# jhollowed/PyTEMDiags

Hardware: AMD Instinct MI355X
Metric: grid-points/sec through full TEM pipeline (ncol*nlev*nt) (higher is better)
Workload: dtype f64; 1 GPU; ne120 (777602 cols) x 72 lev x 30 snapshots per GPU, L=50, 1-degree zonal grid (M=180), ten GM16 Table-A1 outputs; ncol=777602, nlev=72, nt=30, sweeps=latitude-class, single sweep, mirror_paired_sweeps=True

## Files before the change

### include/temx.h

```cpp
#ifndef TEMX_H
#define TEMX_H

#include <stdint.h>

#ifdef __cplusplus
extern "C" {
#endif

typedef struct temx_plan temx_plan;

enum { TEMX_F64 = 0, TEMX_F32 = 1 };

enum {
  TEMX_OK = 0,
  TEMX_EINVAL = -1,
  TEMX_EHIP = -2,
  TEMX_ENOMEM = -3,
  TEMX_ERANK = -4,
  TEMX_ESTATE = -5,
  TEMX_EUNSUPPORTED = -6,
  TEMX_EINTERNAL = -7
};

enum {
  TEMX_DEFER_FINALIZE = 1,
  TEMX_NO_SYMMETRY = 2,
  TEMX_NO_CLASSES = 4,
  TEMX_NO_QR = 8,
  TEMX_LAT_TOL_F32 = 16
};

enum {
  TEMX_OPT_FORM = 1,
  TEMX_OPT_OS_MAP = 2,
  TEMX_OPT_OP_MAP = 3,
  TEMX_OPT_OS_SUBSAMPLE = 4,
  TEMX_OPT_TRACER_ONE_PASS = 5,
  TEMX_OPT_SINGLE_SWEEP_MIN_GROUPS = 6,
  TEMX_OPT_OS_CONTRACT = 7,
  TEMX_OPT_MISSING = 8,
  TEMX_OPT_MIN_COVERAGE = 9,
  TEMX_OPT_MISSING_WEIGHT = 10,
  TEMX_OPT_LAT_BINS = 12,
  TEMX_OPT_BIN_DEGREE = 13,
  TEMX_OPT_OS_SYNC = 11
};
enum {
  TEMX_FORM_AUTO = -1,
  TEMX_FORM_TWO_PASS = 0,
  TEMX_FORM_CLASS_SUMS = 1,
  TEMX_FORM_SINGLE_SWEEP = 2,
  TEMX_FORM_NO_SINGLE_SWEEP = 3,
  TEMX_FORM_MASKED = 4,
  TEMX_FORM_BINNED = 5
};

enum {
  TEMX_MAT_Y0 = 0,
  TEMX_MAT_Y0P = 1,
  TEMX_MAT_GRAM = 2,
  TEMX_MAT_GINV = 3,
  TEMX_MAT_Y0INV = 4,
  TEMX_MAT_GRAM2 = 5,
  TEMX_MAT_GX = 6,
  TEMX_MAT_GSUB = 7,
  TEMX_MAT_COVERAGE = 8
};

enum {
  TEMX_R_VTEM = 0, TEMX_R_OMEGATEM, TEMX_R_WTEM, TEMX_R_PSITEM, TEMX_R_EPFY, TEMX_R_EPFZ,
  TEMX_R_EPDIV, TEMX_R_UTENDEPFD, TEMX_R_UTENDVTEM, TEMX_R_UTENDWTEM, TEMX_NRESULTS
};

enum {
  TEMX_Z_UB = 0, TEMX_Z_VB, TEMX_Z_THETAB, TEMX_Z_WAPB, TEMX_Z_UPVPB, TEMX_Z_UPWAPPB,
  TEMX_Z_VPTPB, TEMX_Z_DUB_DP, TEMX_Z_DTHETAB_DP, TEMX_Z_UBCOSLAT, TEMX_Z_DUBCOSLAT_DLAT,
  TEMX_Z_PSI, TEMX_Z_PSICOSLAT, TEMX_Z_DPSICOSLAT_DLAT, TEMX_Z_DPSI_DP, TEMX_Z_INT_VBDP,
// ... 127 lines not shown
```

### pytemdiags_amd/_lib.py

```python
from __future__ import annotations

import ctypes as C
import os

_HERE = os.path.dirname(os.path.abspath(__file__))
LIB_PATH = os.environ.get("TEMX_LIB") or os.path.join(_HERE, "libtemx.so")

ABI_VERSION = 402
F64, F32 = 0, 1
DEFER_FINALIZE = 1
NO_SYMMETRY = 2
NO_CLASSES = 4
NO_QR = 8
LAT_TOL_F32 = 16
MAT_Y0, MAT_Y0P, MAT_GRAM, MAT_GINV, MAT_Y0INV, MAT_GRAM2, MAT_GX, MAT_GSUB = 0, 1, 2, 3, 4, 5, 6, 7
MAT_COVERAGE = 8
OPT_FORM, OPT_OS_MAP, OPT_OP_MAP, OPT_OS_SUBSAMPLE, OPT_TRACER_ONE_PASS, OPT_SINGLE_SWEEP_MIN_GROUPS, OPT_OS_CONTRACT = 1, 2, 3, 4, 5, 6, 7
OPT_MISSING, OPT_MIN_COVERAGE, OPT_MISSING_WEIGHT = 8, 9, 10
OPT_OS_SYNC = 11
OPT_LAT_BINS, OPT_BIN_DEGREE = 12, 13
LAT_BINS_ALLOWED = (128, 256, 512, 1024, 2048)
LAT_BINS_DEFAULT = 512
MISSING_MODES = {"raise": 0, "mask": 1}
FORM_AUTO, FORM_TWO_PASS, FORM_CLASS_SUMS, FORM_SINGLE_SWEEP, FORM_NO_SINGLE_SWEEP = -1, 0, 1, 2, 3
FORM_MASKED = 4
FORM_BINNED = 5
FORM_NAMES = {FORM_TWO_PASS: "two-pass", FORM_CLASS_SUMS: "class-sums", FORM_SINGLE_SWEEP: "single-sweep",
              FORM_MASKED: "masked", FORM_BINNED: "binned"}
FORMS = {"auto": FORM_AUTO, "two-pass": FORM_TWO_PASS, "class-sums": FORM_CLASS_SUMS,
         "single-sweep": FORM_SINGLE_SWEEP, "no-single-sweep": FORM_NO_SINGLE_SWEEP}

RESULT_NAMES = ("vtem", "omegatem", "wtem", "psitem", "epfy", "epfz", "epdiv",
                "utendepfd", "utendvtem", "utendwtem")
ZONAL_NAMES = ("ub", "vb", "thetab", "wapb", "upvpb", "upwappb", "vptpb", "dub_dp", "dthetab_dp",
               "ubcoslat", "dubcoslat_dlat", "psi", "psicoslat", "dpsicoslat_dlat", "dpsi_dp",
               "int_vbdp")
EDDY_NAMES = ("up", "vp", "thetap", "wapp", "upvp", "upwapp", "vptp")
TRACER_RESULT_NAMES = ("etfy", "etfz", "etdiv", "qtendetfd", "qtendvtem", "qtendwtem")
TRACER_ZONAL_NAMES = ("qb", "qpvpb", "qpwappb", "dqb_dp", "qbcoslat", "dqbcoslat_dlat")
TRACER_EDDY_NAMES = ("qp", "qpvp", "qpwapp")

ERRORS = {0: "TEMX_OK", -1: "TEMX_EINVAL", -2: "TEMX_EHIP", -3: "TEMX_ENOMEM", -4: "TEMX_ERANK",
          -5: "TEMX_ESTATE", -6: "TEMX_EUNSUPPORTED", -7: "TEMX_EINTERNAL"}

_vp, _i, _i64, _dp, _u64 = C.c_void_p, C.c_int, C.c_int64, C.POINTER(C.c_double), C.c_uint64
SIGNATURES = [
    ("temx_version", _i, []),
    ("temx_last_error", C.c_char_p, []),
    ("temx_device_count", _i, []),
    ("temx_plan_create", _i, [C.POINTER(_vp), _i, _i64, _i, _i, _dp, _dp, _i]),
    ("temx_plan_finalize", _i, [_vp, _dp]),
    ("temx_plan_refine", _i, [_vp, _dp]),
# ... 114 lines not shown
```

### pytemdiags_amd/csrc/kernels_op2.hpp

```cpp
#pragma once
#include "kernels_op.hpp"

namespace temx {

template <int NA, int NB>
struct OpwSlot {
  double sd[2][NA][64];
  double y[NB * 16];
};

template <int TBS, int NA>
__device__ __forceinline__ void opw_round(const OpwSlot<NA, 2 * TBS>* slots, int par, int t0, int nbw,
                                          uint32_t yoff, int lane, double (&acc)[NA][(TBS + 1) / 2]) {
  asm volatile("s_waitcnt lgkmcnt(0)\n\ts_barrier" ::: "memory");
#pragma unroll
  for (int j = 0; j < 4; ++j) {
    double b[NA];
#pragma unroll
    for (int f = 0; f < NA; ++f) b[f] = slots[j].sd[par][f][lane];
#pragma unroll
    for (int tl = 0; tl < (TBS + 1) / 2; ++tl)
      if (tl < nbw) {
        const double ya = slots[j].y[(t0 + tl) * 16 + yoff];
#pragma unroll
// ... 548 lines not shown
#endif
template <typename T> struct RowLoad;
template <> struct RowLoad<double> {
  static __device__ __forceinline__ void ld(double& dst, uint32_t voff, uint64_t sbase) {
    asm volatile("global_load_dwordx2 %0, %1, %2 " TEMX_ROWLOAD_MOD : "=v"(dst) : "v"(voff), "s"(sbase) : "memory");
  }
};
template <> struct RowLoad<float> {
  static __device__ __forceinline__ void ld(float& dst, uint32_t voff, uint64_t sbase) {
    asm volatile("global_load_dword %0, %1, %2 " TEMX_ROWLOAD_MOD : "=v"(dst) : "v"(voff), "s"(sbase) : "memory");
  }
};
__device__ __forceinline__ double temx_rcp_count(double n) {
  double r = __builtin_amdgcn_rcp(n);
  return __builtin_fma(__builtin_fma(-n, r, 1.0), r, r);
}
template <int N, typename T>
__device__ __forceinline__ void row_wait(T& a, T& b, T& c, T& d) {
  asm volatile("s_waitcnt vmcnt(%4)" : "+v"(a), "+v"(b), "+v"(c), "+v"(d) : "n"(N) : "memory");
}
template <int N, typename T>
__device__ __forceinline__ void row_wait(T& a, T& b, T& c) {
  asm volatile("s_waitcnt vmcnt(%3)" : "+v"(a), "+v"(b), "+v"(c) : "n"(N) : "memory");
}
template <typename T>
__device__ __forceinline__ void row_touch(T& a) {
  asm volatile("" : "+v"(a)::"memory");
}

constexpr int HANDOFF_LOOKS = 1 << 22;
__device__ __forceinline__ uint32_t handoff_look(const uint32_t* ctr) {
  return __hip_atomic_load(ctr, __ATOMIC_RELAXED, __HIP_MEMORY_SCOPE_WORKGROUP);
}
template <typename T, int TBS, int TBX, int NBR, int PD, int KIND = 0, int SYNC = 0>
__global__ void __launch_bounds__(256, 1)
sweep_osr_kernel(FieldPtrs<4> fp, int64_t D, int K, int KX, const double* __restrict__ ycx,
                 const int4* __restrict__ crow, const int2* __restrict__ csplit,
                 const double* __restrict__ colscale, const double* __restrict__ rho, int K4,
                 double* __restrict__ px, double* __restrict__ pp, int nsplit, int ndt, int* __restrict__ hstat) {
  using KD = OsKind<KIND>;
  constexpr int NF = KD::NF, NFX = KD::NFX, NP = KD::NP;
  constexpr int NBX = 2 * TBX;
  constexpr int YE = NBX * 16;
  constexpr int YJ = (YE + 255) / 256;
  constexpr int MB = CLS_MB;
  constexpr int NCH = 4;
  constexpr int NV = 2 * (NF + NP);
  constexpr int NPR = KD::NPR, NPL = NP - NPR;
  static_assert(NBR <= TBS && TBS <= TBX, "reference degree <= L <= 2L");
  static_assert(YJ <= 2, "Y quarter per thread");
  static_assert((PD - 1) * CLS_MB * KD::NF + (CLS_MB - 1) * KD::NF + 2 <= 63, "the ring is counted in vmcnt (6 bits)");
  extern __shared__ double lds[];
  int split, dq;
  if (!wg_work((ndt + 3) / 4, nsplit, split, dq)) return;
  const int tid = threadIdx.x;
  const int wave = uniform_wave(), lane = tid & 63;
  const int c = lane & 15, g = lane >> 4;
  const int64_t colr = (int64_t)dq * 64 + lane < D ? (int64_t)dq * 64 + lane : D - 1;
  const uint32_t colb32 = (uint32_t)colr * (uint32_t)sizeof(T);
  const int dt = dq * 4 + wave;
  const int64_t d = (int64_t)dt * 16 + c;
  const bool dvalid = dt < ndt && d < D;
  const int64_t dcl = dvalid ? d : D - 1;
  const int b0 = __builtin_amdgcn_readfirstlane(csplit[split].x);
  const int b1 = __builtin_amdgcn_readfirstlane(csplit[split + 1].x);
  int grp = __builtin_amdgcn_readfirstlane(csplit[split].y);
  const uint32_t aoff_p = (uint32_t)(g * 4 + (lane & 3));
  const uint32_t aoff_r = (uint32_t)((lane & 3) * 4 + g);
  double* ybase = lds;
  double* cn = lds + 2 * YE;
  double* cb = lds + 2 * YE + 16 + wave * (NF * 2 * NBR * 64) + lane;
  double* apl = lds + 2 * YE + 16 + 4 * (NF * 2 * NBR * 64) + wave * (NPL * 2 * TBS * 64) + lane;
  double* ex = lds + 2 * YE + 16 + 4 * (NF * 2 * NBR * 64) + 4 * (NPL * 2 * TBS * 64);
  double* exw = ex + wave * 64 + lane;
  const double* exr = ex + g * 64 + wave * 16 + c;
  uint32_t* hctr = reinterpret_cast<uint32_t*>(ex + NV * 256);
  const double sth = (KD::TF >= 0 && colscale != nullptr) ? colscale[colr] : 1.0;
  if constexpr (SYNC != 0) {
    if (tid < 2) hctr[tid] = 0u;
    __syncthreads();
  }
#pragma unroll
  for (int i = 0; i < NPL * 2 * TBS; ++i) apl[i * 64] = 0.0;
  double apr[NPR > 0 ? NPR : 1][2 * TBS];
// ... 1 lines not shown
  for (int k = 0; k < (NPR > 0 ? NPR : 1); ++k)
#pragma unroll
    for (int t = 0; t < 2 * TBS; ++t) apr[k][t] = 0.0;
#pragma unroll
  for (int f = 0; f < NF; ++f)
#pragma unroll
    for (int tb = 0; tb < 2 * NBR; ++tb) {
      const int l = tb < NBR ? 2 * (4 * tb + g) : 2 * (4 * (tb - NBR) + g) + 1;
      const double v = rho[((int64_t)f * K4 + (l < K ? l : K - 1)) * D + dcl];
      cb[(f * 2 * NBR + tb) * 64] = l < K ? v : 0.0;
    }
  uint64_t fbase[NF];
#pragma unroll
  for (int f = 0; f < NF; ++f) fbase[f] = reinterpret_cast<uint64_t>(fp.p[f]);
  { double sth_ready = sth; asm volatile("" : "+v"(sth_ready)); }

  double ax[NFX][NBX];
#pragma unroll
  for (int f = 0; f < NFX; ++f)
#pragma unroll
    for (int t = 0; t < NBX; ++t) ax[f][t] = 0.0;
  double s[NF], q[NP], x0[NF], cnt = 0.0;
  double sN[NF], qN[NP], x0N[NF], cntN = 0.0;
#pragma unroll
  for (int f = 0; f < NF; ++f) s[f] = x0[f] = sN[f] = x0N[f] = 0.0;
#pragma unroll
  for (int k = 0; k < NP; ++k) q[k] = qN[k] = 0.0;
  bool north_open = false, prev_south = false;
  const uint32_t rowbytes = (uint32_t)D * (uint32_t)sizeof(T);

  T xb[PD][MB][NF];
  int er[PD][MB];
  double ys[YJ];
  const uint32_t yoff32[2] = {(uint32_t)(tid < YE ? tid : 0) * 8u, (uint32_t)(tid + 256 < YE ? tid + 256 : 0) * 8u};
  auto load_ys = [&](int gi) __attribute__((always_inline)) {
#pragma unroll
    for (int j = 0; j < YJ; ++j) RowLoad<double>::ld(ys[j], yoff32[j], reinterpret_cast<uint64_t>(ycx) + (uint64_t)gi * (YE * 8));
  };
  auto issue = [&](auto pc, const int4 rv) __attribute__((always_inline)) {
    constexpr int P = decltype(pc)::value;
    er[P][0] = rv.x; er[P][1] = rv.y; er[P][2] = rv.z; er[P][3] = rv.w;
#pragma unroll
    for (int j = 0; j < MB; ++j) {
      const uint64_t off = (uint64_t)(uint32_t)(er[P][j] & CLS_ROWMASK) * rowbytes;
#pragma unroll
      for (int f = 0; f < NF; ++f) RowLoad<T>::ld(xb[P][j][f], colb32, fbase[f] + off);
    }
  };
  double dS[NFX][2], dP[NP][2];
  const double* yprev = ybase;
  int ycur = 0;
  int left = 0;
#pragma unroll
  for (int f = 0; f < NFX; ++f) dS[f][0] = dS[f][1] = 0.0;
#pragma unroll
  for (int k = 0; k < NP; ++k) dP[k][0] = dP[k][1] = 0.0;
  auto pending_chunk = [&](auto cc) __attribute__((always_inline)) {
    constexpr int C = decltype(cc)::value;
#pragma unroll
    for (int t = C * NBX / NCH; t < (C + 1) * NBX / NCH; ++t) {
      const double ya = yprev[t * 16 + aoff_p];
#pragma unroll
      for (int f = 0; f < NFX; ++f) ax[f][t] = TEMX_MFMA4(ya, dS[f][t < TBX ? 0 : 1], ax[f][t]);
      const int tp = t < TBX ? t : t - TBX;
      if (tp < TBS) {
        const int ta = t < TBX ? tp : TBS + tp;
#pragma unroll
        for (int k = 0; k < NPR; ++k) apr[k][ta] = TEMX_MFMA4(ya, dP[k][t < TBX ? 0 : 1], apr[k][ta]);
        if constexpr (NPL > 0) {
          double v[NPL > 0 ? NPL : 1];
// ... 53 lines not shown
      m2[1][f] -= E[f] - O[f];
    }
#pragma unroll
    for (int f = 0; f < NFX; ++f) {
      const double SNf = nN * m2[0][f], SSf = nS * m2[1][f];
      dS[f][0] = SNf + SSf;
      dS[f][1] = SNf - SSf;
    }
#pragma unroll
    for (int k = 0; k < NP; ++k) {
      const double PNk = c2[0][k] + nN * m2[0][KD::pa(k)] * m2[0][KD::pb(k)];
      const double PSk = c2[1][k] + nS * m2[1][KD::pa(k)] * m2[1][KD::pb(k)];
      dP[k][0] = PNk + PSk;
      dP[k][1] = PNk - PSk;
    }
    yprev = yw;
    left = NCH;
  };
  uint32_t hgen = 0;
  bool hpend = false;
  int hfail = 0;
  const double* ypend = ybase;
  auto handoff_wait = [&](const uint32_t* ctr, uint32_t seen, uint32_t need, int code) __attribute__((always_inline)) {
    seen = (uint32_t)__builtin_amdgcn_readfirstlane((int)seen);
    if (seen >= need || hfail != 0) return;
#pragma unroll 1
    for (int n = 0; n < HANDOFF_LOOKS; ++n) {
      __builtin_amdgcn_s_sleep(1);
      seen = (uint32_t)__builtin_amdgcn_readfirstlane((int)handoff_look(ctr));
      if (seen >= need) return;
    }
    hfail = code;
  };
  int4 rn;
  auto step = [&](auto posc, int b) __attribute__((always_inline)) {
    constexpr int POS = decltype(posc)::value % NCH;
    constexpr int P = decltype(posc)::value % PD;
    uint32_t seen = 0;
    if constexpr (SYNC != 0) {
      if (hpend) seen = handoff_look(&hctr[0]);
    }
    {
      const int4 r1 = rn;
      rn = crow[(int64_t)(b + PD) * 4 + wave];
      issue(std::integral_constant<int, (P + PD - 1) % PD>{}, r1);
    }
    if constexpr (SYNC != 0) {
      if (hpend) {
        if (left > 0)
          static_for<NCH>([&](auto cc) __attribute__((always_inline)) {
            if (((decltype(cc)::value - POS) & (NCH - 1)) < left) pending_chunk(cc);
          });
        handoff_wait(&hctr[0], seen, 4u * hgen, 1);
        tile_role(ypend);
        hpend = false;
      }
    }
    if (left > 0) {
      if (!(TEMX_OS_SKIP & 1)) pending_chunk(std::integral_constant<int, POS>{});
      --left;
    }
    static_assert(NF == 4 || NF == 3, "row_wait has forms for 3 and 4 fields");
    static_for<MB>([&](auto jc) __attribute__((always_inline)) {
      constexpr int j = decltype(jc)::value;
      constexpr int NW = (PD - 1) * MB * NF + (MB - 1 - j) * NF;
      if constexpr (NF == 4) row_wait<NW>(xb[P][j][0], xb[P][j][1], xb[P][j][2], xb[P][j][3]);
      else row_wait<NW>(xb[P][j][0], xb[P][j][1], xb[P][j][2]);
    });
#pragma unroll
    for (int j = 0; j < YJ; ++j) row_touch(ys[j]);
    const int fl = er[P][0] >> 27;
    const bool south = (fl & (CLS_SOUTH << 1)) != 0;
    if ((fl & (CLS_FIRST << 1)) || (south && !prev_south)) {
      if (south && north_open) park_north();
      north_open = !south;
#pragma unroll
      for (int f = 0; f < NF; ++f) x0[f] = (double)xb[P][0][f];
    }
    prev_south = south;
#pragma unroll
    for (int j = 0; j < ((TEMX_OS_SKIP & 4) ? 0 : MB); ++j) {
      const double w = er[P][j] < 0 ? 0.0 : 1.0;
      double dx[NF];
#pragma unroll
      for (int f = 0; f < NF; ++f) dx[f] = (double)xb[P][j][f] - x0[f];
#pragma unroll
      for (int f = 0; f < NF; ++f) s[f] += w * dx[f];
#pragma unroll
      for (int k = 0; k < NP; ++k) q[k] += (w * dx[KD::pa(k)]) * dx[KD::pb(k)];
      cnt += w;
    }
    if (fl & (CLS_LAST << 1)) {
      prev_south = false;
      if (north_open) park_north();
      north_open = false;
      uint32_t seen_done = 0;
      if constexpr (SYNC == 0) {
        if (left > 0)
          static_for<NCH>([&](auto cc) __attribute__((always_inline)) {
            if (((decltype(cc)::value - POS - 1) & (NCH - 1)) < left) pending_chunk(cc);
          });
      } else {
        seen_done = handoff_look(&hctr[1]);
      }
      const double rnN = cntN > 0.0 ? temx_rcp_count(cntN) : 0.0, rnS = cnt > 0.0 ? temx_rcp_count(cnt) : 0.0;
      double val[NV];
#pragma unroll
      for (int f = 0; f < NF; ++f) {
        const double sc = f == KD::TF ? sth : 1.0;
        val[f] = (sN[f] * rnN + x0N[f]) * sc;
        val[NF + NP + f] = (s[f] * rnS + x0[f]) * sc;
      }
#pragma unroll
      for (int k = 0; k < NP; ++k) {
        const double sc = k == KD::TP ? sth : 1.0;
        val[NF + k] = (qN[k] - sN[KD::pa(k)] * sN[KD::pb(k)] * rnN) * sc;
        val[2 * NF + NP + k] = (q[k] - s[KD::pa(k)] * s[KD::pb(k)] * rnS) * sc;
      }
      if constexpr (SYNC == 0) {
        if (!(TEMX_OS_SKIP & 8)) asm volatile("s_waitcnt lgkmcnt(0)\n\ts_barrier" ::: "memory");
      } else {
        handoff_wait(&hctr[1], seen_done, 4u * hgen, 2);
      }
      ycur ^= 1;
      double* yw = ybase + ycur * YE;
#pragma unroll
      for (int v = 0; v < NV; ++v) exw[v * 256] = val[v];
      if (lane == 0) {
        cn[wave] = cntN;
        cn[4 + wave] = cnt;
      }
#pragma unroll
      for (int j = 0; j < YJ; ++j)
        if (tid + 256 * j < YE) yw[tid + 256 * j] = ys[j];
      if constexpr (SYNC == 0) {
        if (!(TEMX_OS_SKIP & 8)) asm volatile("s_waitcnt lgkmcnt(0)\n\ts_barrier" ::: "memory");
      } else {
        asm volatile("s_waitcnt lgkmcnt(0)" ::: "memory");
        if (lane == 0) __hip_atomic_fetch_add(&hctr[0], 1u, __ATOMIC_RELAXED, __HIP_MEMORY_SCOPE_WORKGROUP);
        ++hgen;
        hpend = true;
        ypend = yw;
      }
      ++grp;
      load_ys(grp);
      if constexpr (SYNC == 0) tile_role(yw);
#pragma unroll
      for (int f = 0; f < NF; ++f) s[f] = sN[f] = 0.0;
#pragma unroll
      for (int k = 0; k < NP; ++k) q[k] = qN[k] = 0.0;
      cnt = cntN = 0.0;
    }
  };

  if (b0 < b1) {
    load_ys(grp);
    rn = crow[(int64_t)b0 * 4 + wave];
    static_for<PD - 1>([&](auto kc) __attribute__((always_inline)) {
      constexpr int k = decltype(kc)::value;
      const int4 r0 = rn;
      rn = crow[(int64_t)(b0 + k + 1) * 4 + wave];
      issue(kc, r0);
    });
    constexpr int UNR = PD % 4 == 0 ? PD : PD % 2 == 0 ? 2 * PD : 4 * PD;
    for (int b = b0; b < b1; b += UNR)
      static_for<UNR>([&](auto kc) __attribute__((always_inline)) {
        constexpr int k = decltype(kc)::value;
        if (k == 0 || b + k < b1) step(kc, b + k);
      });
    asm volatile("s_waitcnt vmcnt(0)" ::: "memory");
  }
  if constexpr (SYNC != 0) {
    if (hpend) {
      if (left > 0) {
        const int first = (b1 - b0) & (NCH - 1);
        static_for<NCH>([&](auto cc) __attribute__((always_inline)) {
          if (((decltype(cc)::value - first) & (NCH - 1)) < left) pending_chunk(cc);
        });
      }
      handoff_wait(&hctr[0], handoff_look(&hctr[0]), 4u * hgen, 1);
      tile_role(ypend);
    }
    if (hfail != 0 && lane == 0) atomicOr(hstat, hfail);
  }
  if (left > 0) {
    const int first = (b1 - b0) & (NCH - 1);
    static_for<NCH>([&](auto cc) __attribute__((always_inline)) {
      if (((decltype(cc)::value - first) & (NCH - 1)) < left) pending_chunk(cc);
    });
  }
  if (dvalid) {
#pragma unroll
    for (int f = 0; f < NFX; ++f)
#pragma unroll
      for (int t = 0; t < NBX; ++t) {
        const int l = symx_harm<TBX>(t, g);
        if (l < (pp != nullptr ? KX : K4)) px[(((int64_t)split * NFX + f) * KX + l) * D + d] = ax[f][t];
      }
#pragma unroll
    for (int k = 0; k < NP; ++k)
#pragma unroll
      for (int t = 0; t < 2 * TBS; ++t) {
        const int l = sym_harm<TBS>(t, g);
        if (pp != nullptr && l < K) pp[(((int64_t)split * NP + k) * K + l) * D + d] = k < NPR ? apr[k < NPR ? k : 0][t] : apl[((k < NPR ? 0 : k - NPR) * 2 * TBS + t) * 64];
      }
  }
}

#ifndef TEMX_OS2_STAGGER
#define TEMX_OS2_STAGGER 0
#endif
#ifndef TEMX_OS2_ACC32
#define TEMX_OS2_ACC32 1
#endif
// ... 703 lines not shown
```

### pytemdiags_amd/csrc/temx.hip

```cpp
#include "../../include/temx.h"
#include "../../include/temx_vert.h"
#include "../../include/temx_layout.h"
#include "../../include/temx_ingest.h"
#include "../../include/temx_clim.h"
#include "../../include/temx_mtracer.h"
#include "../../include/temx_nclim.h"
#include "../../include/temx_gclim.h"
#include "../include/temx_mgclim.h"
#include "../include/temx_wave.h"
#include "../include/temx_tfilt.h"

#include <hip/hip_runtime.h>

#include <algorithm>
#include <cmath>
#include <cstdarg>
#include <cstdio>
#include <cstdlib>
#include <cstring>
#include <map>
#include <mutex>
#include <new>
#include <stdexcept>
#include <string>
// ... 115 lines not shown
  Split sp_proj1;
  bool sym = false;
  int TBS = 0;
  int64_t npair = 0, npg = 0, npg_alloc = 0;
  DevBuf rows, ysym;
  Split sp_sproj4, sp_sproj1, sp_seddy;
  Split sp_proj4, sp_eddy;
  bool cls = false;
  int64_t cgroups = 0, cbatches = 0, ncls = 0;
  int64_t cls_max_side = 0;
  std::vector<int> gbatch0;
  DevBuf crow, ycls;
  std::map<int, DevBuf> csplits;
  Split sp_cproj4, sp_cproj1, sp_ceddy, sp_cflux;
  bool os_built = false, os_on = false;
  bool os_valid = false;
  DevBuf Axq, rho_t;
  int TBX = 0, KX = 0, KR = 0, NQ = 0;
  std::vector<double> h_xc, h_cnt;
  std::vector<int> h_crow;
  std::vector<int> sgbatch0;
  int64_t sgroups = 0, sbatches = 0;
  DevBuf ycx, ycx_s, crow_s, rho, rho0, gaunt , wq2, Gx, Gsinv, Ax , Axs ;
  std::vector<double> h_G_own;
  std::vector<double> h_Gx_own;
  std::vector<double> h_Gx, h_Gs;
  std::vector<double> h_T, h_Ginv, h_G, h_Yq;
  DevBuf oscblk, osAt, osAb, osAtq, osAbq, Bqp;
  OscMats osc{};
  bool osc_lds = false;
  int opt_os_contract = -1;
  bool os_barrier = false;
  int opt_os_sync = -1;
  int os_keep = 32;
  int64_t tD = 0, tnt = 0, tt0 = 0;
  int opt_form = -1, opt_os_map = -1, opt_op_map = -1, opt_tracer_one_pass = -1, opt_single_sweep_min_groups = -1;
  bool os_tile = false, op_tile = false;
  bool no_qr = false;
  DevBuf side_crow[2][2], side_gfirst[2][2];
  std::map<int, DevBuf> csplits_s;
  Split sp_os, sp_os_s;
  Split sp_copw;
  bool lcls = false, lone = false, xb_valid = false;
  DevBuf ycls_l, pbuf;
  int64_t ycls_lstride = 0;
  Split sp_lflux;
  bool onepass = false, op_valid = false;
  bool c4_valid = false;
  DevBuf csum, ccnt;
  DevBuf Pq;
  DevBuf csq, Pq2;
  bool tq_valid = false;
  DevBuf partial;
  DevBuf opB, opC;
  int opt_missing = 0, opt_min_cov = 500, opt_miss_w = 10;
  bool miss_built = false;
  bool miss_valid = false;
  int64_t miss_cov_D = -1;
  int NE = 0, NQM = 0;
  DevBuf eblk;
  DevBuf mtab;
  DevBuf mB, mC, mCcov, mcov, mZ;
  bool mt_valid = false;
  DevBuf mtB, mtB2, mtC, mtCcov, mtz;
  int opt_lat_bins = 0;
  int bin_J = 0, bin_KP = 0;
// ... 648 lines not shown
  constexpr int NBR = OS_NBR;
  constexpr int PDv = sizeof(T) == 4 ? 4 : 2;
  constexpr int DF = TEMX_OS_DEFER;
  const bool tile_map = pl->os_tile;
  double* px = partial;
  double* pp = sub ? nullptr : partial + (int64_t)sp.nsplit * KD::NFX * pl->KX * pl->D;
  int rc = TEMX_OK;
  const bool listed = dispatch_strict(OsPairs{}, pl->TBS, pl->TBX, rc, [&](auto pair) {
    constexpr int TBSv = decltype(pair)::first, TBXv = decltype(pair)::second;
    if constexpr (KIND == 3) {
      if (tile_map) return fail(TEMX_EUNSUPPORTED, "two tracers per sweep: row-map sweeps only");
    }
    if constexpr (KIND != 3) if (tile_map) {
      constexpr size_t lds = sweep_os_lds(TBSv, TBXv, KD::NF, KD::NP, KD::NPR, DF);
      return launch_lds<sweep_os_kernel<T, TBSv, TBXv, NBR, PDv, KIND, DF>>(pl->device, grid, block, lds, st, fp, pl->D,
          pl->K, pl->KX, sub ? pl->ycx_s.d() : pl->ycx.d(), static_cast<const int4*>(sub ? pl->crow_s.p : pl->crow.p), cuts,
          pl->colscale.d(), rho, pl->KR, px, pp, sp.nsplit, sp.ndt);
    }
    if (sizeof(T) == 4) {
      if (pl->cls_max_side > 8 * TEMX_F32_SIDE_CAP)
        return fail(TEMX_EUNSUPPORTED, "single sweep of fp32 fields: a latitude class of this plan has %lld members on one "
                    "side, and the sweep sums a side in fp32; create the plan with TEMX_LAT_TOL_F32",
                    (long long)pl->cls_max_side);
      constexpr size_t lds = sweep_os2_lds(TBSv, TBXv, KD::NF, KD::NP, KD::NPR, DF);
      const int si = sub ? 1 : 0;
      return launch_lds<sweep_os2_kernel<float, TBSv, TBXv, NBR, 2, KIND>>(
          pl->device, grid, dim3(512), lds, st, fp, pl->D, pl->K, pl->KX, sub ? pl->ycx_s.d() : pl->ycx.d(),
          static_cast<const int4*>(pl->side_crow[si][0].p), static_cast<const int4*>(pl->side_crow[si][1].p),
          static_cast<const int*>(pl->side_gfirst[si][0].p), static_cast<const int*>(pl->side_gfirst[si][1].p),
          cuts, pl->colscale.d(), rho, pl->KR, px, pp, sp.nsplit, sp.ndt);
    }
    constexpr size_t lds = sweep_osr_lds(TBSv, TBXv, KD::NF, KD::NP, KD::NPR, DF);
    static_assert(lds <= 163840, "the single sweep's workgroup fits the LDS of a compute unit");
    auto go = [&](auto handoff) {
      return launch_lds<sweep_osr_kernel<double, TBSv, TBXv, NBR, 2, KIND, decltype(handoff)::value>>(pl->device, grid,
          block, lds, st, fp, pl->D, pl->K, pl->KX, sub ? pl->ycx_s.d() : pl->ycx.d(),
          static_cast<const int4*>(sub ? pl->crow_s.p : pl->crow.p), cuts, pl->colscale.d(), rho, pl->KR, px, pp, sp.nsplit,
          sp.ndt, static_cast<int*>(pl->flag.p) + 1);
    };
    return pl->os_barrier ? go(Int<0>{}) : go(Int<1>{});
  });
  return listed ? rc : fail(TEMX_EUNSUPPORTED, "single-sweep form: no instantiation for L = %d", pl->L);
}

template <int KIND>
static int launch_sweep_os(temx_plan* pl, const FieldPtrs<4>& fp, int dtype, bool sub, const double* rho, double* partial,
                           const Split& sp, hipStream_t st) {
  return dtype == TEMX_F64 ? launch_sweep_os_t<double, KIND>(pl, fp, sub, rho, partial, sp, st)
                           : launch_sweep_os_t<float, KIND>(pl, fp, sub, rho, partial, sp, st);
}

static bool os_supported(const temx_plan* pl) {
  return os_supported(pl->cls, pl->large, pl->weighted, pl->qbasis, !pl->h_crow.empty(), pl->TBS, pl->L);
}

static bool os_active(const temx_plan* pl, int dtype) {
  (void)dtype;
  return pl->os_on;
}

static void set_tail(temx_plan* pl, int64_t t0, int64_t nts) {
  if (pl->tt0 != t0 || pl->tnt != nts) pl->c4_valid = pl->os_valid = pl->op_valid = pl->tq_valid = pl->xb_valid = false;
  pl->tt0 = t0;
  pl->tnt = nts;
  pl->tD = (int64_t)pl->nlev * nts;
}
static inline bool tail_is_whole(const temx_plan* pl) { return pl->tt0 == 0 && pl->tnt == pl->nt; }

static int tem_stage3_impl(temx_plan* pl, const double* B3, double* results, double* zonal, hipStream_t st);
static int tem_epilogue(temx_plan* pl, double* results, double* zonal, hipStream_t st);
static int bin_project_op(temx_plan* pl, const void* A, int dtype, int64_t D, double* B, hipStream_t st);
static int bin_zonal_mean(temx_plan* pl, const void* A, int dtype, int64_t D, double* out, int native, hipStream_t st);
static int miss_check(const temx_plan* pl);
// ... 1291 lines not shown
  if (!pl || !B || !out) return fail(TEMX_EINVAL, "null argument");
  if (!pl->finalized) return fail(TEMX_ESTATE, "plan not finalised");
  HIPCHK(hipSetDevice(pl->device));
  int rc;
  if (!native) return launch_solve(pl, B, 1, D, nullptr, out, S_(stream));
  if ((rc = pl->opC.ensure((size_t)pl->K4 * D * 8))) return rc;
  if ((rc = launch_solve(pl, B, 1, D, pl->opC.d(), nullptr, S_(stream)))) return rc;
  return launch_recon(pl, D, pl->opC.d(), out, S_(stream));
} TEMX_CATCH

int temx_zonal_mean(temx_plan* pl, const void* A, int dtype, int64_t D, double* out, int native,
                    void* stream) try {
  if (!pl || !A || !out) return fail(TEMX_EINVAL, "null argument");
  if (!pl->finalized) return fail(TEMX_ESTATE, "plan not finalised");
  if (miss_mode(pl)) return miss_zonal_mean(pl, A, dtype, D, out, native, S_(stream));
  if (bin_mode(pl)) return bin_zonal_mean(pl, A, dtype, D, out, native, S_(stream));
  int rc = pl->opB.ensure((size_t)pl->K * std::max<int64_t>(D, 1) * 8);
  if (rc) return rc;
  if ((rc = temx_project(pl, A, dtype, D, pl->opB.d(), stream))) return rc;
  return temx_zonal_mean_from_sums(pl, pl->opB.d(), D, out, native, stream);
} TEMX_CATCH

static FormChoice form_choice(const temx_plan* pl) {
  return form_choice(pl->opt_form, bin_mode(pl), getenv("TEMX_TWO_PASS"), getenv("TEMX_ONE_PASS"), getenv("TEMX_SINGLE_SWEEP"));
}
static bool tile_map(int opt, const char* env) {
  if (const char* e = getenv(env)) return !strcmp(e, "tile");
  return opt == 1;
}
static bool os_barrier_wanted(const temx_plan* pl) {
  if (const char* e = getenv("TEMX_OS_SYNC")) return !strcmp(e, "barrier");
  return pl->opt_os_sync == 1;
}
static bool tracer_one_pass_wanted(const temx_plan* pl) {
  if (const char* e = getenv("TEMX_TRACER_ONE_PASS")) return e[0] == '1';
  return pl->opt_tracer_one_pass == 1;
}

static int bin_check(const temx_plan* pl);
static int bin_set_tem(temx_plan* pl);

int temx_plan_configure(temx_plan* pl, int option, int value) try {
  if (!pl) return fail(TEMX_EINVAL, "null plan");
  switch (option) {
    case TEMX_OPT_FORM:
      if (value < -1 || value > TEMX_FORM_NO_SINGLE_SWEEP) return fail(TEMX_EINVAL, "TEMX_OPT_FORM: unknown form %d", value);
      pl->opt_form = value;
      break;
    case TEMX_OPT_OS_MAP: pl->opt_os_map = value; break;
    case TEMX_OPT_OP_MAP: pl->opt_op_map = value; break;
    case TEMX_OPT_TRACER_ONE_PASS: pl->opt_tracer_one_pass = value; break;
    case TEMX_OPT_OS_SUBSAMPLE:
      if (value < 4) return fail(TEMX_EINVAL, "TEMX_OPT_OS_SUBSAMPLE: at least 4 class-groups");
      if (pl->os_built && value != pl->os_keep) return fail(TEMX_ESTATE, "the single-sweep tables of this plan are built: set the subsample before temx_plan_set_tem");
      pl->os_keep = value;
      break;
    case TEMX_OPT_SINGLE_SWEEP_MIN_GROUPS: pl->opt_single_sweep_min_groups = value; break;
    case TEMX_OPT_OS_CONTRACT: pl->opt_os_contract = value; break;
    case TEMX_OPT_MISSING:
      if (value != 0 && value != 1) return fail(TEMX_EINVAL, "TEMX_OPT_MISSING: 0 (raise) or 1 (mask), got %d", value);
      if (value == 1) {
        if (bin_mode(pl)) return fail(TEMX_EUNSUPPORTED, "missing-value mode is not available while latitude bins are in effect (TEMX_OPT_LAT_BINS)");
        if (int rc = miss_check(pl)) return rc;
      }
      pl->opt_missing = value;
      pl->miss_valid = false;
      break;
    case TEMX_OPT_MIN_COVERAGE:
      if (value < 0 || value > 1000) return fail(TEMX_EINVAL, "TEMX_OPT_MIN_COVERAGE: per mille in 0..1000, got %d", value);
      pl->opt_min_cov = value;
      break;
    case TEMX_OPT_MISSING_WEIGHT:
      if (value < 4 || value > 14) return fail(TEMX_EINVAL, "TEMX_OPT_MISSING_WEIGHT: tau = 10^-value, value in 4..14, got %d", value);
      pl->opt_miss_w = value;
      break;
    case TEMX_OPT_OS_SYNC:
      if (value != 0 && value != 1) return fail(TEMX_EINVAL, "TEMX_OPT_OS_SYNC: 0 (flags) or 1 (barriers), got %d", value);
      pl->opt_os_sync = value;
      break;
    case TEMX_OPT_LAT_BINS: {
      const int B = value == -1 ? BIN_DEFAULT : value;
      if (B != 0) {
        if (!bin_count_ok(B)) return fail(TEMX_EINVAL, "TEMX_OPT_LAT_BINS: 0 (off), -1 (default, %d) or one of 128, 256, 512, 1024, 2048, got %d", BIN_DEFAULT, value);
        if (int rc = bin_check(pl)) return rc;
        if (bin_degree(pl->L, B) == 0)
          return fail(TEMX_EINVAL, "TEMX_OPT_LAT_BINS: (L, B) = (%d, %d): no Chebyshev degree up to %d keeps the basis rows to %.0e; use more bins",
                      pl->L, B, BIN_MAX_DEGREE, BIN_BOUND);
      }
      pl->opt_lat_bins = B;
      pl->bin_J = B ? bin_degree(pl->L, B) : 0;
      break;
    }
    case TEMX_OPT_BIN_DEGREE: return fail(TEMX_EINVAL, "TEMX_OPT_BIN_DEGREE is chosen by the library (read it with temx_plan_option)");
    default: return fail(TEMX_EINVAL, "unknown option %d", option);
  }
  pl->tem = false;
  return TEMX_OK;
} TEMX_CATCH

int temx_plan_option(const temx_plan* pl, int option) try {
  if (!pl) return -1;
  switch (option) {
    case TEMX_OPT_FORM:
      if (miss_mode(pl)) return TEMX_FORM_MASKED;
      if (bin_mode(pl)) return TEMX_FORM_BINNED;
      return pl->os_on ? TEMX_FORM_SINGLE_SWEEP : ((pl->cls && pl->onepass) || (pl->lcls && pl->lone) ? TEMX_FORM_CLASS_SUMS : TEMX_FORM_TWO_PASS);
    case TEMX_OPT_OS_MAP: return tile_map(pl->opt_os_map, "TEMX_OS_MAP") ? 1 : 0;
    case TEMX_OPT_OP_MAP: return tile_map(pl->opt_op_map, "TEMX_OP_MAP") ? 1 : 0;
    case TEMX_OPT_TRACER_ONE_PASS: return tracer_one_pass_wanted(pl) ? 1 : 0;
    case TEMX_OPT_OS_SUBSAMPLE: return pl->os_keep;
    case TEMX_OPT_SINGLE_SWEEP_MIN_GROUPS: return pl->opt_single_sweep_min_groups;
    case TEMX_OPT_OS_CONTRACT: return pl->osc_lds ? 1 : 0;
    case TEMX_OPT_MISSING: return pl->opt_missing;
    case TEMX_OPT_MIN_COVERAGE: return pl->opt_min_cov;
    case TEMX_OPT_MISSING_WEIGHT: return pl->opt_miss_w;
    case TEMX_OPT_OS_SYNC: return os_barrier_wanted(pl) ? 1 : 0;
    case TEMX_OPT_LAT_BINS: return pl->opt_lat_bins;
    case TEMX_OPT_BIN_DEGREE: return pl->bin_J;
    default: return -1;
  }
} TEMX_CATCH

static bool mem_free(size_t* fr) {
  size_t tot = 0;
  return hipMemGetInfo(fr, &tot) == hipSuccess;
}

static int set_tem_large_cls(temx_plan* pl, const TemDims& d, const FormChoice& fc) {
  const LargeClsLayout l = tem_large_cls_layout(d, fc);
  size_t fr = 0;
  if (!(l.eligible && mem_free(&fr) && fits(l.csum, pl->csum.bytes, fr, l.pbuf) &&
        alloc_write_stream(pl->csum, l.csum) == TEMX_OK && pl->pbuf.ensure(l.pbuf) == TEMX_OK))
    return TEMX_OK;
  int rc;
  HIPCHK(hipMemset(pl->csum.p, 0, pl->csum.bytes));
  HIPCHK(hipMemset(pl->pbuf.p, 0, pl->pbuf.bytes));
  pl->sp_cproj4 = l.sp_cproj4;
  pl->sp_cflux = l.sp_cflux;
  pl->sp_lflux = l.sp_lflux;
  if ((rc = pl->partial.ensure(l.partial))) return rc;
  if ((rc = pl->Bs.ensure(l.Bs))) return rc;
  const int2* cuts_unused = nullptr;
  if ((rc = class_cuts_dev(pl, pl->sp_cproj4.nsplit, &cuts_unused, true))) return rc;
  pl->lone = true;
  return TEMX_OK;
}

static int set_tem_single_sweep(temx_plan* pl, const TemDims& d) {
  int rc = build_os_tables(pl);
// ... 47 lines not shown
  for (int nsub : {pl->sp_cproj4.nsplit, pl->sp_cproj1.nsplit, pl->sp_ceddy.nsplit * (8 / d.edpw())})
    if ((rc = class_cuts_dev(pl, nsub, &cuts_unused))) return rc;
  return TEMX_OK;
}

static int set_tem_sym(temx_plan* pl, const TemDims& d) {
  const SymLayout s = tem_sym_layout(d);
  pl->sp_sproj4 = s.sp_sproj4;
  pl->sp_sproj1 = s.sp_sproj1;
  pl->sp_seddy = s.sp_seddy;
  return pl->partial.ensure(s.partial);
}

int temx_plan_set_tem(temx_plan* pl, int nlev, int64_t nt, const double* p_pa_host, double p0) try {
  if (!pl || !p_pa_host) return fail(TEMX_EINVAL, "null argument");
  if (nlev < 2 || nt < 1) return fail(TEMX_EINVAL, "need nlev >= 2 and nt >= 1");
  if ((int64_t)nlev * nt >= ((int64_t)1 << 28)) return fail(TEMX_EINVAL, "nlev*nt must be < 2^28");
  if (pl->M < 2) return fail(TEMX_EINVAL, "need at least 2 zonal-mean latitudes");
  HIPCHK(hipSetDevice(pl->device));
  std::vector<double> p(p_pa_host, p_pa_host + nlev);
  for (int j = 1; j < nlev; ++j)
    if (!(p[j] > p[j - 1])) return fail(TEMX_EINVAL, "pressure must be strictly ascending (front end flips)");
  pl->tem = false;
  pl->onepass = pl->lone = pl->op_valid = pl->xb_valid = pl->tq_valid = false;
  pl->os_on = pl->os_valid = false;
  pl->miss_valid = pl->mt_valid = false;
  pl->os_tile = tile_map(pl->opt_os_map, "TEMX_OS_MAP");
  {
    const char* e = getenv("TEMX_OS_CONTRACT");
    pl->osc_lds = e ? !strcmp(e, "lds") : pl->opt_os_contract == 1;
  }
  pl->op_tile = tile_map(pl->opt_op_map, "TEMX_OP_MAP");
  pl->os_barrier = os_barrier_wanted(pl);
  pl->nlev = nlev;
  pl->nt = nt;
  pl->D = (int64_t)nlev * nt;
  pl->tD = pl->D;
  pl->tnt = nt;
  pl->tt0 = 0;
  pl->p0 = p0;
  int rc;
  const TemTables tt = tem_tables(p, nt, p0, pl->lat_out_deg);
  if ((rc = upload(pl->p, p))) return rc;
  if ((rc = upload(pl->pg, tt.pg))) return rc;
  if ((rc = upload(pl->lg, tt.lg))) return rc;
  if ((rc = upload(pl->coslat, tt.coslat))) return rc;
  if ((rc = upload(pl->fcor, tt.fcor))) return rc;
  if ((rc = upload(pl->colscale, tt.colscale))) return rc;

  const TemDims d = tem_dims(pl);
  const FormChoice fc = form_choice(pl);
  const BaseLayout b = tem_base_layout(d);
  pl->sp_proj4 = b.sp_proj4;
  pl->sp_eddy = b.sp_eddy;
  pl->sp_proj1 = b.sp_proj1;
  if ((rc = pl->partial.ensure(b.partial))) return rc;
  if ((rc = pl->B4.ensure(b.B4))) return rc;
  if ((rc = pl->B3.ensure(b.B3))) return rc;
  if ((rc = pl->C4.ensure(b.C4))) return rc;
  if ((rc = pl->zb.ensure(b.zb))) return rc;
  if ((rc = pl->partial.ensure(b.partial_unfused))) return rc;
  if (pl->lcls && (rc = set_tem_large_cls(pl, d, fc))) return rc;
  if (pl->cls && (rc = set_tem_cls(pl, d, fc))) return rc;
  if (pl->sym && (rc = set_tem_sym(pl, d))) return rc;
  if (bin_mode(pl) && (rc = bin_set_tem(pl))) return rc;
  pl->tem = true;
// ... 1600 lines not shown
```

### pytemdiags_amd/engine.py

```python
from __future__ import annotations

import ctypes as C

import numpy as np
import torch

from . import _lib
from ._lib import check

_DT = {torch.float64: _lib.F64, torch.float32: _lib.F32}


def _ptr(t):
    return C.c_void_p(t.data_ptr())


def _dbl(a):
    a = np.ascontiguousarray(a, dtype=np.float64)
    return a, a.ctypes.data_as(C.POINTER(C.c_double))


def lat_bins_value(lat_bins):
    if lat_bins is None or lat_bins is False:
        return 0
# ... 23 lines not shown
        check(self.lib.temx_plan_create(C.byref(self._h), self.device_index, self.N, self.L, self.M,
                                        plat, plat_out, (_lib.DEFER_FINALIZE if defer_finalize else 0)
                                        | (0 if symmetry else _lib.NO_SYMMETRY)
                                        | (0 if classes else _lib.NO_CLASSES)
                                        | (0 if qr else _lib.NO_QR)
                                        | (_lib.LAT_TOL_F32 if fp32_fields else 0)))
        if form is not None:
            self.configure(form=form)
        if lat_bins is not None:
            self.configure(lat_bins=lat_bins)

    @property
    def paired(self):
        return bool(self.lib.temx_plan_is_paired(self._h))

    @property
    def sweep_mode(self):
        return int(self.lib.temx_plan_sweep_mode(self._h))

    @property
    def one_pass(self):
        return bool(self.lib.temx_plan_one_pass(self._h))

    @property
    def single_sweep(self):
        return bool(self.lib.temx_plan_single_sweep(self._h))

    @property
    def tracer_one_pass(self):
        return self.one_pass and self.option(_lib.OPT_TRACER_ONE_PASS) == 1

    def configure(self, form=None, os_map=None, op_map=None, os_subsample=None, tracer_one_pass=None,
                  single_sweep_min_groups=None, os_contract=None, missing=None, min_coverage=None,
                  missing_weight=None, os_sync=None, lat_bins=None):
        def put(opt, val):
            check(self.lib.temx_plan_configure(self._h, opt, int(val)))
        if missing is not None:
            if missing not in _lib.MISSING_MODES:
                raise ValueError("missing must be 'raise' or 'mask', got %r" % (missing,))
            put(_lib.OPT_MISSING, _lib.MISSING_MODES[missing])
        if min_coverage is not None:
            mc = float(min_coverage)
            if not 0.0 <= mc <= 1.0:
                raise ValueError("min_coverage must lie in [0, 1], got %r" % (min_coverage,))
            put(_lib.OPT_MIN_COVERAGE, int(round(mc * 1000)))
        if missing_weight is not None:
            e = -np.log10(float(missing_weight))
            if not (float(missing_weight) > 0 and abs(e - round(e)) < 1e-9 and 4 <= round(e) <= 14):
                raise ValueError("missing_weight must be 10^-n with n in 4..14, got %r" % (missing_weight,))
            put(_lib.OPT_MISSING_WEIGHT, int(round(e)))
        if form is not None:
            put(_lib.OPT_FORM, _lib.FORMS[form] if isinstance(form, str) else form)
            self.form_requested = form
        for opt, val in ((_lib.OPT_OS_MAP, os_map), (_lib.OPT_OP_MAP, op_map)):
            if val is not None:
                put(opt, {"row": 0, "tile": 1}[val] if isinstance(val, str) else val)
        if os_subsample is not None:
            put(_lib.OPT_OS_SUBSAMPLE, os_subsample)
        if tracer_one_pass is not None:
            put(_lib.OPT_TRACER_ONE_PASS, 1 if tracer_one_pass else 0)
        if single_sweep_min_groups is not None:
            put(_lib.OPT_SINGLE_SWEEP_MIN_GROUPS, single_sweep_min_groups)
        if os_contract is not None:
            put(_lib.OPT_OS_CONTRACT, {"mfma": 0, "lds": 1}[os_contract] if isinstance(os_contract, str) else os_contract)
        if lat_bins is not None:
            put(_lib.OPT_LAT_BINS, lat_bins_value(lat_bins))
        if os_sync is not None:
            put(_lib.OPT_OS_SYNC, {"flags": 0, "barrier": 1}[os_sync] if isinstance(os_sync, str) else os_sync)
        self.nlev = self.nt = self.D = None

    def option(self, opt):
        return int(self.lib.temx_plan_option(self._h, int(opt)))

    @property
    def lat_bins(self):
        return self.option(_lib.OPT_LAT_BINS)

    @property
    def bin_degree(self):
        return self.option(_lib.OPT_BIN_DEGREE)

    @property
    def sweep_form(self):
        return _lib.FORM_NAMES.get(self.option(_lib.OPT_FORM), "two-pass")

    @property
    def missing(self):
        return "mask" if self.option(_lib.OPT_MISSING) == 1 else "raise"

    def coverage(self):
        D = getattr(self, "_cov_D", None) or self.D or 1
        out = torch.empty((self.M, D), dtype=torch.float64, device=self.device)
        check(self.lib.temx_get_matrix(self._h, _lib.MAT_COVERAGE, _ptr(out), self._stream()))
        return out

    def close(self):
        if getattr(self, "_h", None) is not None and self._h.value:
            self.lib.temx_plan_destroy(self._h)
            self._h = C.c_void_p()

    def __del__(self):
# ... 639 lines not shown
```

Before: 189.3 billion grid-points/s.

## Defer single-sweep group hand-over production until after next chunk issue

Adds a 'late' hand-over variant to the flag-synchronised single-sweep kernel, now the default. When a latitude group closes, the kernel no longer computes and publishes its zonal statistics and Y rows on the spot. It records a pending production, prefetches the next group's Y into a separate register set, and performs the production at the next step, after the following row loads are issued. The goal is to hide the hand-over wait and LDS writes behind in-flight memory traffic. In exchange it uses extra registers, adds scalar state, and needs more careful ordering at the kernel tail.

Result: no change. 191.7 billion grid-points/s, median of 6 (+1.3%).

```diff
diff --git a/include/temx.h b/include/temx.h
--- a/include/temx.h
+++ b/include/temx.h
@@ -43,6 +43,7 @@
   TEMX_OPT_MISSING_WEIGHT = 10,
   TEMX_OPT_LAT_BINS = 12,
   TEMX_OPT_BIN_DEGREE = 13,
+  TEMX_OPT_OS_HANDOVER = 14,
   TEMX_OPT_OS_SYNC = 11
 };
 enum {
diff --git a/pytemdiags_amd/_lib.py b/pytemdiags_amd/_lib.py
--- a/pytemdiags_amd/_lib.py
+++ b/pytemdiags_amd/_lib.py
@@ -18,6 +18,7 @@
 OPT_FORM, OPT_OS_MAP, OPT_OP_MAP, OPT_OS_SUBSAMPLE, OPT_TRACER_ONE_PASS, OPT_SINGLE_SWEEP_MIN_GROUPS, OPT_OS_CONTRACT = 1, 2, 3, 4, 5, 6, 7
 OPT_MISSING, OPT_MIN_COVERAGE, OPT_MISSING_WEIGHT = 8, 9, 10
 OPT_OS_SYNC = 11
+OPT_OS_HANDOVER = 14
 OPT_LAT_BINS, OPT_BIN_DEGREE = 12, 13
 LAT_BINS_ALLOWED = (128, 256, 512, 1024, 2048)
 LAT_BINS_DEFAULT = 512
diff --git a/pytemdiags_amd/csrc/kernels_op2.hpp b/pytemdiags_amd/csrc/kernels_op2.hpp
--- a/pytemdiags_amd/csrc/kernels_op2.hpp
+++ b/pytemdiags_amd/csrc/kernels_op2.hpp
@@ -604,7 +604,7 @@
 __device__ __forceinline__ uint32_t handoff_look(const uint32_t* ctr) {
   return __hip_atomic_load(ctr, __ATOMIC_RELAXED, __HIP_MEMORY_SCOPE_WORKGROUP);
 }
-template <typename T, int TBS, int TBX, int NBR, int PD, int KIND = 0, int SYNC = 0>
+template <typename T, int TBS, int TBX, int NBR, int PD, int KIND = 0, int SYNC = 0, int LATE = 0>
 __global__ void __launch_bounds__(256, 1)
 sweep_osr_kernel(FieldPtrs<4> fp, int64_t D, int K, int KX, const double* __restrict__ ycx,
                  const int4* __restrict__ crow, const int2* __restrict__ csplit,
@@ -622,6 +622,7 @@
   static_assert(NBR <= TBS && TBS <= TBX, "reference degree <= L <= 2L");
   static_assert(YJ <= 2, "Y quarter per thread");
   static_assert((PD - 1) * CLS_MB * KD::NF + (CLS_MB - 1) * KD::NF + 2 <= 63, "the ring is counted in vmcnt (6 bits)");
+  static_assert(LATE == 0 || SYNC != 0, "the late hand-over is a form of the flag hand-over");
   extern __shared__ double lds[];
   int split, dq;
   if (!wg_work((ndt + 3) / 4, nsplit, split, dq)) return;
@@ -689,10 +690,11 @@
   T xb[PD][MB][NF];
   int er[PD][MB];
   double ys[YJ];
+  double ysn[LATE ? YJ : 1];
   const uint32_t yoff32[2] = {(uint32_t)(tid < YE ? tid : 0) * 8u, (uint32_t)(tid + 256 < YE ? tid + 256 : 0) * 8u};
   auto load_ys = [&](int gi) __attribute__((always_inline)) {
 #pragma unroll
-    for (int j = 0; j < YJ; ++j) RowLoad<double>::ld(ys[j], yoff32[j], reinterpret_cast<uint64_t>(ycx) + (uint64_t)gi * (YE * 8));
+    for (int j = 0; j < YJ; ++j) RowLoad<double>::ld(LATE ? ysn[LATE ? j : 0] : ys[j], yoff32[j], reinterpret_cast<uint64_t>(ycx) + (uint64_t)gi * (YE * 8));
   };
   auto issue = [&](auto pc, const int4 rv) __attribute__((always_inline)) {
     constexpr int P = decltype(pc)::value;
@@ -812,13 +814,67 @@
     }
     hfail = code;
   };
+  auto produce = [&](uint32_t seen_done) __attribute__((always_inline)) {
+    const double rnN = cntN > 0.0 ? temx_rcp_count(cntN) : 0.0, rnS = cnt > 0.0 ? temx_rcp_count(cnt) : 0.0;
+    double val[NV];
+#pragma unroll
+    for (int f = 0; f < NF; ++f) {
+      const double sc = f == KD::TF ? sth : 1.0;
+      val[f] = (sN[f] * rnN + x0N[f]) * sc;
+      val[NF + NP + f] = (s[f] * rnS + x0[f]) * sc;
+    }
+#pragma unroll
+    for (int k = 0; k < NP; ++k) {
+      const double sc = k == KD::TP ? sth : 1.0;
+      val[NF + k] = (qN[k] - sN[KD::pa(k)] * sN[KD::pb(k)] * rnN) * sc;
+      val[2 * NF + NP + k] = (q[k] - s[KD::pa(k)] * s[KD::pb(k)] * rnS) * sc;
+    }
+    if constexpr (SYNC == 0) {
+      if (!(TEMX_OS_SKIP & 8)) asm volatile("s_waitcnt lgkmcnt(0)\n\ts_barrier" ::: "memory");
+    } else {
+      handoff_wait(&hctr[1], seen_done, 4u * hgen, 2);
+    }
+    ycur ^= 1;
+    double* yw = ybase + ycur * YE;
+#pragma unroll
+    for (int v = 0; v < NV; ++v) exw[v * 256] = val[v];
+    if (lane == 0) {
+      cn[wave] = cntN;
+      cn[4 + wave] = cnt;
+    }
+#pragma unroll
+    for (int j = 0; j < YJ; ++j)
+      if (tid + 256 * j < YE) yw[tid + 256 * j] = ys[j];
+    if constexpr (SYNC == 0) {
+      if (!(TEMX_OS_SKIP & 8)) asm volatile("s_waitcnt lgkmcnt(0)\n\ts_barrier" ::: "memory");
+    } else {
+      asm volatile("s_waitcnt lgkmcnt(0)" ::: "memory");
+      if (lane == 0) __hip_atomic_fetch_add(&hctr[0], 1u, __ATOMIC_RELAXED, __HIP_MEMORY_SCOPE_WORKGROUP);
+      ++hgen;
+      hpend = true;
+      ypend = yw;
+    }
+    return yw;
+  };
+  auto zero_sums = [&]() __attribute__((always_inline)) {
+#pragma unroll
+    for (int f = 0; f < NF; ++f) s[f] = sN[f] = 0.0;
+#pragma unroll
+    for (int k = 0; k < NP; ++k) q[k] = qN[k] = 0.0;
+    cnt = cntN = 0.0;
+  };
+  int hprod = 0;
   int4 rn;
   auto step = [&](auto posc, int b) __attribute__((always_inline)) {
     constexpr int POS = decltype(posc)::value % NCH;
     constexpr int P = decltype(posc)::value % PD;
-    uint32_t seen = 0;
+    uint32_t seen = 0, seen_late = 0;
     if constexpr (SYNC != 0) {
       if (hpend) seen = handoff_look(&hctr[0]);
+      if constexpr (LATE != 0) {
+        asm volatile("" : "+s"(hprod));
+        if (hprod) seen_late = handoff_look(&hctr[1]);
+      }
     }
     {
       const int4 r1 = rn;
@@ -834,6 +890,16 @@
         handoff_wait(&hctr[0], seen, 4u * hgen, 1);
         tile_role(ypend);
         hpend = false;
+        if constexpr (LATE != 0) {
+          if (hprod) seen_late = handoff_look(&hctr[1]);
+        }
+      }
+      if constexpr (LATE != 0) {
+        if (hprod) {
+          produce(seen_late);
+          zero_sums();
+          hprod = 0;
+        }
       }
     }
     if (left > 0) {
@@ -847,8 +913,16 @@
       if constexpr (NF == 4) row_wait<NW>(xb[P][j][0], xb[P][j][1], xb[P][j][2], xb[P][j][3]);
       else row_wait<NW>(xb[P][j][0], xb[P][j][1], xb[P][j][2]);
     });
-#pragma unroll
-    for (int j = 0; j < YJ; ++j) row_touch(ys[j]);
+    if constexpr (LATE != 0) {
+#pragma unroll
+      for (int j = 0; j < YJ; ++j) {
+        row_touch(ysn[j]);
+        asm volatile("v_mov_b64 %0, %1" : "=v"(ys[j]) : "v"(ysn[j]));
+      }
+    } else {
+#pragma unroll
+      for (int j = 0; j < YJ; ++j) row_touch(ys[j]);
+    }
     const int fl = er[P][0] >> 27;
     const bool south = (fl & (CLS_SOUTH << 1)) != 0;
     if ((fl & (CLS_FIRST << 1)) || (south && !prev_south)) {
@@ -874,62 +948,30 @@
       prev_south = false;
       if (north_open) park_north();
       north_open = false;
-      uint32_t seen_done = 0;
-      if constexpr (SYNC == 0) {
-        if (left > 0)
-          static_for<NCH>([&](auto cc) __attribute__((always_inline)) {
-            if (((decltype(cc)::value - POS - 1) & (NCH - 1)) < left) pending_chunk(cc);
-          });
+      if constexpr (LATE != 0) {
+        hprod = 1;
+        ++grp;
+        load_ys(grp);
+        int no = north_open, ps = prev_south;
+        asm volatile("" : "+s"(no), "+s"(ps));
+        north_open = no != 0;
+        prev_south = ps != 0;
       } else {
-        seen_done = handoff_look(&hctr[1]);
-      }
-      const double rnN = cntN > 0.0 ? temx_rcp_count(cntN) : 0.0, rnS = cnt > 0.0 ? temx_rcp_count(cnt) : 0.0;
-      double val[NV];
-#pragma unroll
-      for (int f = 0; f < NF; ++f) {
-        const double sc = f == KD::TF ? sth : 1.0;
-        val[f] = (sN[f] * rnN + x0N[f]) * sc;
-        val[NF + NP + f] = (s[f] * rnS + x0[f]) * sc;
-      }
-#pragma unroll
-      for (int k = 0; k < NP; ++k) {
-        const double sc = k == KD::TP ? sth : 1.0;
-        val[NF + k] = (qN[k] - sN[KD::pa(k)] * sN[KD::pb(k)] * rnN) * sc;
-        val[2 * NF + NP + k] = (q[k] - s[KD::pa(k)] * s[KD::pb(k)] * rnS) * sc;
-      }
-      if constexpr (SYNC == 0) {
-        if (!(TEMX_OS_SKIP & 8)) asm volatile("s_waitcnt lgkmcnt(0)\n\ts_barrier" ::: "memory");
-      } else {
-        handoff_wait(&hctr[1], seen_done, 4u * hgen, 2);
-      }
-      ycur ^= 1;
-      double* yw = ybase + ycur * YE;
-#pragma unroll
-      for (int v = 0; v < NV; ++v) exw[v * 256] = val[v];
-      if (lane == 0) {
-        cn[wave] = cntN;
-        cn[4 + wave] = cnt;
-      }
-#pragma unroll
-      for (int j = 0; j < YJ; ++j)
-        if (tid + 256 * j < YE) yw[tid + 256 * j] = ys[j];
-      if constexpr (SYNC == 0) {
-        if (!(TEMX_OS_SKIP & 8)) asm volatile("s_waitcnt lgkmcnt(0)\n\ts_barrier" ::: "memory");
-      } else {
-        asm volatile("s_waitcnt lgkmcnt(0)" ::: "memory");
-        if (lane == 0) __hip_atomic_fetch_add(&hctr[0], 1u, __ATOMIC_RELAXED, __HIP_MEMORY_SCOPE_WORKGROUP);
-        ++hgen;
-        hpend = true;
-        ypend = yw;
-      }
-      ++grp;
-      load_ys(grp);
-      if constexpr (SYNC == 0) tile_role(yw);
-#pragma unroll
-      for (int f = 0; f < NF; ++f) s[f] = sN[f] = 0.0;
-#pragma unroll
-      for (int k = 0; k < NP; ++k) q[k] = qN[k] = 0.0;
-      cnt = cntN = 0.0;
+        uint32_t seen_done = 0;
+        if constexpr (SYNC == 0) {
+          if (left > 0)
+            static_for<NCH>([&](auto cc) __attribute__((always_inline)) {
+              if (((decltype(cc)::value - POS - 1) & (NCH - 1)) < left) pending_chunk(cc);
+            });
+        } else {
+          seen_done = handoff_look(&hctr[1]);
+        }
+        double* yw = produce(seen_done);
+        ++grp;
+        load_ys(grp);
+        if constexpr (SYNC == 0) tile_role(yw);
+        zero_sums();
+      }
     }
   };
 
@@ -951,7 +993,7 @@
     asm volatile("s_waitcnt vmcnt(0)" ::: "memory");
   }
   if constexpr (SYNC != 0) {
-    if (hpend) {
+    auto take_last = [&]() __attribute__((always_inline)) {
       if (left > 0) {
         const int first = (b1 - b0) & (NCH - 1);
         static_for<NCH>([&](auto cc) __attribute__((always_inline)) {
@@ -960,6 +1002,14 @@
       }
       handoff_wait(&hctr[0], handoff_look(&hctr[0]), 4u * hgen, 1);
       tile_role(ypend);
+      hpend = false;
+    };
+    if (hpend) take_last();
+    if constexpr (LATE != 0) {
+      if (hprod) {
+        produce(handoff_look(&hctr[1]));
+        take_last();
+      }
     }
     if (hfail != 0 && lane == 0) atomicOr(hstat, hfail);
   }
diff --git a/pytemdiags_amd/csrc/temx.hip b/pytemdiags_amd/csrc/temx.hip
--- a/pytemdiags_amd/csrc/temx.hip
+++ b/pytemdiags_amd/csrc/temx.hip
@@ -171,6 +171,8 @@
   int opt_os_contract = -1;
   bool os_barrier = false;
   int opt_os_sync = -1;
+  bool os_late = false;
+  int opt_os_handover = -1;
   int os_keep = 32;
   int64_t tD = 0, tnt = 0, tt0 = 0;
   int opt_form = -1, opt_os_map = -1, opt_op_map = -1, opt_tracer_one_pass = -1, opt_single_sweep_min_groups = -1;
@@ -885,13 +887,13 @@
     }
     constexpr size_t lds = sweep_osr_lds(TBSv, TBXv, KD::NF, KD::NP, KD::NPR, DF);
     static_assert(lds <= 163840, "the single sweep's workgroup fits the LDS of a compute unit");
-    auto go = [&](auto handoff) {
-      return launch_lds<sweep_osr_kernel<double, TBSv, TBXv, NBR, 2, KIND, decltype(handoff)::value>>(pl->device, grid,
+    auto go = [&](auto handoff, auto late) {
+      return launch_lds<sweep_osr_kernel<double, TBSv, TBXv, NBR, 2, KIND, decltype(handoff)::value, decltype(late)::value>>(pl->device, grid,
           block, lds, st, fp, pl->D, pl->K, pl->KX, sub ? pl->ycx_s.d() : pl->ycx.d(),
           static_cast<const int4*>(sub ? pl->crow_s.p : pl->crow.p), cuts, pl->colscale.d(), rho, pl->KR, px, pp, sp.nsplit,
           sp.ndt, static_cast<int*>(pl->flag.p) + 1);
     };
-    return pl->os_barrier ? go(Int<0>{}) : go(Int<1>{});
+    return pl->os_barrier ? go(Int<0>{}, Int<0>{}) : pl->os_late ? go(Int<1>{}, Int<1>{}) : go(Int<1>{}, Int<0>{});
   });
   return listed ? rc : fail(TEMX_EUNSUPPORTED, "single-sweep form: no instantiation for L = %d", pl->L);
 }
@@ -2249,6 +2251,14 @@
   if (const char* e = getenv("TEMX_OS_SYNC")) return !strcmp(e, "barrier");
   return pl->opt_os_sync == 1;
 }
+constexpr int OS_HANDOVER_DEFAULT = 1;
+static bool os_late_wanted(const temx_plan* pl) {
+  if (const char* e = getenv("TEMX_OS_HANDOVER")) {
+    if (!strcmp(e, "late")) return true;
+    if (!strcmp(e, "early")) return false;
+  }
+  return (pl->opt_os_handover < 0 ? OS_HANDOVER_DEFAULT : pl->opt_os_handover) == 1;
+}
 static bool tracer_one_pass_wanted(const temx_plan* pl) {
   if (const char* e = getenv("TEMX_TRACER_ONE_PASS")) return e[0] == '1';
   return pl->opt_tracer_one_pass == 1;
@@ -2295,6 +2305,10 @@
       if (value != 0 && value != 1) return fail(TEMX_EINVAL, "TEMX_OPT_OS_SYNC: 0 (flags) or 1 (barriers), got %d", value);
       pl->opt_os_sync = value;
       break;
+    case TEMX_OPT_OS_HANDOVER:
+      if (value != 0 && value != 1) return fail(TEMX_EINVAL, "TEMX_OPT_OS_HANDOVER: 0 (early) or 1 (late), got %d", value);
+      pl->opt_os_handover = value;
+      break;
     case TEMX_OPT_LAT_BINS: {
       const int B = value == -1 ? BIN_DEFAULT : value;
       if (B != 0) {
@@ -2332,6 +2346,7 @@
     case TEMX_OPT_MIN_COVERAGE: return pl->opt_min_cov;
     case TEMX_OPT_MISSING_WEIGHT: return pl->opt_miss_w;
     case TEMX_OPT_OS_SYNC: return os_barrier_wanted(pl) ? 1 : 0;
+    case TEMX_OPT_OS_HANDOVER: return os_late_wanted(pl) ? 1 : 0;
     case TEMX_OPT_LAT_BINS: return pl->opt_lat_bins;
     case TEMX_OPT_BIN_DEGREE: return pl->bin_J;
     default: return -1;
@@ -2445,6 +2460,7 @@
   }
   pl->op_tile = tile_map(pl->opt_op_map, "TEMX_OP_MAP");
   pl->os_barrier = os_barrier_wanted(pl);
+  pl->os_late = os_late_wanted(pl);
   pl->nlev = nlev;
   pl->nt = nt;
   pl->D = (int64_t)nlev * nt;
diff --git a/pytemdiags_amd/engine.py b/pytemdiags_amd/engine.py
--- a/pytemdiags_amd/engine.py
+++ b/pytemdiags_amd/engine.py
@@ -79,7 +79,7 @@
 
     def configure(self, form=None, os_map=None, op_map=None, os_subsample=None, tracer_one_pass=None,
                   single_sweep_min_groups=None, os_contract=None, missing=None, min_coverage=None,
-                  missing_weight=None, os_sync=None, lat_bins=None):
+                  missing_weight=None, os_sync=None, lat_bins=None, os_handover=None):
         def put(opt, val):
             check(self.lib.temx_plan_configure(self._h, opt, int(val)))
         if missing is not None:
@@ -114,6 +114,8 @@
             put(_lib.OPT_LAT_BINS, lat_bins_value(lat_bins))
         if os_sync is not None:
             put(_lib.OPT_OS_SYNC, {"flags": 0, "barrier": 1}[os_sync] if isinstance(os_sync, str) else os_sync)
+        if os_handover is not None:
+            put(_lib.OPT_OS_HANDOVER, {"early": 0, "late": 1}[os_handover] if isinstance(os_handover, str) else os_handover)
         self.nlev = self.nt = self.D = None
 
     def option(self, opt):
```
